# afb2001/path_planner

Hardware: AMD Instinct MI355X
Metric: Dubins edges costed/sec on 2048x2048 grid (higher is better)
Workload: dtype f64; 1 GPU; cfg3_2048_10pct_65536_obst16; grid=2048x2048 @0.1m, 10% blocked, samples_per_iter_per_gpu=65536, samples_per_iter_total=65536, dynamic_obstacles=16, obstacle_placement=uniform in the map (SURVEY 8d), seed 3, ribbons=5, heuristic=TspPointRobotNoSplitKRibbons K=2, edges_per_iter_per_gpu=236140

## Files before the change

### path_planner_amd/csrc/pp_k_common.h

```cpp
#pragma once
#include "../../include/ppgpu.h"
#include "pp_device.h"

struct __attribute__((aligned(128))) PPLaunchWords {
    unsigned need_big;
    unsigned live_count;
    unsigned hw_count;
    unsigned defer_count[PP_HL_MAX_N + 1];
    unsigned sweep_count;
    unsigned swept_total;
};
static_assert(sizeof(PPLaunchWords) == 128, "the launch counters share one 128-byte line");
static_assert(offsetof(PPLaunchWords, sweep_count) % 8 == 0 && offsetof(PPLaunchWords, swept_total) == offsetof(PPLaunchWords, sweep_count) + 4,
              "pp_k_mark_sweeps adds to sweep_count (low half) and swept_total (high half) with one 64-bit atomic");
__device__ __forceinline__ unsigned long long* pp_sweep_counters(PPLaunchWords* w) { return reinterpret_cast<unsigned long long*>(&w->sweep_count); }

struct PPParams {
    double max_speed, slow_speed, rho, rho_cov, horizon, tmin, inc_d, sst, ribw, cpf, tpf;
    double inv_inc_d;
    int heuristic, tsp_k;
    int fuse_h;
    int quiet_finish;
    int lane_split;
    int defer_h;
    double h_rho;
    PPGrid grid;
    const PPObst* obst; int n_obst; int obst_model;
    const ppgpu_vertex* verts; const double* ribbons; const double* tgrid; int ng; int nverts;
    const double* sx; const double* sy; const double* sh; long long n_samples;
    const unsigned long long* edges; long long n_edges;
    long long total_edges;
    const ppgpu_wrapper_edge* wedges;
    int v0, nv; long long s0, ns; unsigned cfg_mask; int per;
    ppgpu_edge_result* out; double* child; int stride;
    long long e_base, ws_base;
    struct PPEdgeSetup* setup;
    unsigned short* track_hits;
    unsigned long long* track_eq;
    unsigned* track_chunk_hits;
    double* track_pen;
    double* track_chunk_pen;
    struct PPTrackSummary* track_summary;
    unsigned char* track_skip;
    int2* track_far;
    unsigned long long* work;
    PPLaunchWords* words;
    int reset_words;
    unsigned* live_list;
    unsigned* defer_list;
    struct PPCoverState* cover_state;
    unsigned* hw_list;
    int ngp, nch;
    unsigned* share_head;
    unsigned* share_of;
    int approach_list;
    unsigned* sweep_list;
};

#define PP_SETUP_MALFORMED 1u
#define PP_SETUP_COLOCATED 2u
#define PP_SETUP_SHARED 4u
#define PP_SETUP_NO_SWEEP (PP_SETUP_MALFORMED | PP_SETUP_COLOCATED | PP_SETUP_SHARED)
#define PP_SHARE_KEYS 8
#define PP_SHARE_NONE 0xffffffffu
#define PP_FAR_DONE (-2)
#define PP_SHARE_UNSWEPT 0xfffffffeu
struct PPEdgeSetupBody {
    PPSegBase seg[3];
    double p0, p1, p2, hi1;
    double qx, qy, rho, rho_inv, length;
    double wStart, wEnd, speed;
    double approx;
    unsigned long long omask;
    int type;
    unsigned vi, cbits, sflags;
    double srcH;
};
struct __attribute__((aligned(128))) PPEdgeSetup : PPEdgeSetupBody {};
static_assert(sizeof(PPEdgeSetup) == 256 && sizeof(PPEdgeSetupBody) == 256, "PPEdgeSetup is sized for two 128-byte lines");
template <bool TAB = false>
__device__ __forceinline__ void pp_setup_seg_pose(const PPEdgeSetupBody* S, int i, double tprime, double p0, double p1, int word, double& ux, double& uy, double& uth) {
    const PPSegBase* g = &S->seg[i];
    pp_curve_seg<TAB>(pp_word_seg_type(word, i), (tprime - pp_seg_o1(i, p0)) - pp_seg_o2(i, p1), g->bx, g->by, g->bth, g->sb, g->cb, ux, uy, uth);
}
template <bool TAB = false>
__device__ __forceinline__ void pp_setup_seg_pose(const PPEdgeSetupBody* S, int i, double tprime, double& ux, double& uy, double& uth) {
    pp_setup_seg_pose<TAB>(S, i, tprime, S->p0, S->p1, S->type, ux, uy, uth);
}
#define PP_SETUP_GLOBAL_WORDS 32
#define PP_SETUP_WORDS 32
#define PP_SETUP_LDS_STRIDE 33
static_assert(sizeof(PPEdgeSetup) == 8 * PP_SETUP_GLOBAL_WORDS && sizeof(PPEdgeSetupBody) == 8 * PP_SETUP_WORDS, "the LDS staging of the skip planner copies whole records");

__global__ __launch_bounds__(256) void pp_k_grid_row_clear(const uint32_t* bits, int rows, int cols, int wpr, unsigned char* rowclear) {
    const long long i = (long long)blockIdx.x * 256 + threadIdx.x;
    if (i >= (long long)rows * cols) return;
    const int r = (int)(i / cols), c = (int)(i - (long long)r * cols);
    const uint32_t* row = bits + (size_t)r * wpr;
    int d = 0;
    for (; d < PP_CLEAR_CAP; d++) {
        const int a = c - d, b = c + d;
        if (a < 0 || b >= cols) break;
        if (((row[a >> 5] >> (a & 31)) | (row[b >> 5] >> (b & 31))) & 1u) break;
    }
    rowclear[i] = (unsigned char)d;
}
__global__ __launch_bounds__(256) void pp_k_grid_clear(const unsigned char* rowclear, int rows, int cols, unsigned char* clearance) {
    const long long i = (long long)blockIdx.x * 256 + threadIdx.x;
    if (i >= (long long)rows * cols) return;
    const int r = (int)(i / cols), c = (int)(i - (long long)r * cols);
    int best = rowclear[i];
    for (int dy = 1; dy < best; dy++) {
        const int up = r + dy, dn = r - dy;
        int m = dy;
        if (up < rows && dn >= 0) {
            const int ru = rowclear[(size_t)up * cols + c], rd = rowclear[(size_t)dn * cols + c];
            m = max(dy, min(ru, rd));
        }
        best = min(best, m);
    }
    clearance[i] = (unsigned char)best;
}

#define PP_TG_SEG 2048
__global__ __launch_bounds__(64) void pp_k_time_grid(const ppgpu_vertex* verts, int nverts, double sst, double inc_d, double max_speed,
                                                    int ng, double* tgrid) {
    __shared__ double seg[PP_TG_SEG];
    const int v = blockIdx.x;
    if (v >= nverts) return;
    const int lane = threadIdx.x;
    double timeIncrement = inc_d / max_speed;
    double t = verts[v].time;
    double timeSinceStart = t - sst;
    double timeNudge = fmod(timeSinceStart, timeIncrement);
    t += timeNudge;
    double* row = tgrid + (size_t)v * ng;
    int s = 0;
    for (int tries = 0; s < ng && tries < 8; tries++) {
        const double c = (t + timeIncrement) - t;
        int firstBad = ng;
        for (int k0 = s; k0 < ng; k0 += 64) {
            const int k = k0 + lane;
            const double val = t + (double)(k - s) * c;
            const double nxt = t + (double)(k + 1 - s) * c;
            if (k < ng) row[k] = val;
            const bool bad = (k < ng - 1) && !(val + timeIncrement == nxt);
            const unsigned long long m = __ballot(bad);
            if (m != 0ull) { firstBad = k0 + (int)__builtin_ctzll(m); break; }
        }
// ... 90 lines not shown
```

### path_planner_amd/csrc/pp_k_solve.h

```cpp
#pragma once
#ifndef PP_CR_SOLVE
#define PP_CR_SOLVE true
#endif
#ifndef PP_SOLVE_MIN_WAVES
#define PP_SOLVE_MIN_WAVES 1
#endif
__device__ __forceinline__ bool pp_edge_shareable(const PPParams& p, const PPCurve& cv, int type, unsigned sflags, unsigned cbits,
                                                  double wStart, double wEnd, double speed) {
    if (type < 0 || (sflags & (PP_SETUP_MALFORMED | PP_SETUP_COLOCATED)) || cbits >= 4u) return false;
    const double bound = p.horizon + 1e-12 + p.sst;
    if (wEnd < bound) return false;
    const double dist = (bound - wStart) * speed;
    if (!(dist <= cv.length)) return false;
    const double tprime = (cv.rho_inv != 0.0) ? dist * cv.rho_inv : dist / cv.rho;
    return tprime < cv.p0;
}
__device__ __forceinline__ unsigned pp_share_key(unsigned vi, unsigned cbits, int type) {
    return vi * PP_SHARE_KEYS + (cbits & 3u) * 2u + (pp_word_seg_type(type, 0) == 0 ? 0u : 1u);
}
__device__ __forceinline__ void pp_share_elect(const PPParams& p, bool member, unsigned key, unsigned pos) {
    bool pend = false;
    if (member) pend = pos < __hip_atomic_load(p.share_head + key, __ATOMIC_RELAXED, __HIP_MEMORY_SCOPE_AGENT);
    unsigned long long m;
    while ((m = __ballot(pend)) != 0ull) {
        const int leader = __ffsll((long long)m) - 1;
        const unsigned k0 = (unsigned)__builtin_amdgcn_readlane((int)key, leader);
        if (pp_lane() == leader) atomicMin(p.share_head + k0, pos);
        if (key == k0) pend = false;
    }
}

template <bool ALL_WORDS>
__device__ __forceinline__ void pp_solve_edges_body(const PPParams& p) {
    const long long e = (long long)blockIdx.x * 256 + threadIdx.x;
    pp_launch_reset(p, e);
    if (e >= p.n_edges) return;
    long long e2 = -1;
    if (!p.wedges && !p.edges) {
        const long long Q = p.total_edges / p.per;
        const int r = (int)((p.e_base + e) / Q);
        unsigned m = p.cfg_mask;
        for (int i = 0; i < p.per - 1 - r; i++) m &= m - 1;
        const unsigned c = (unsigned)(__ffs((int)m) - 1), c2 = c ^ PPGPU_EDGE_SLOW;
        if ((p.cfg_mask >> c2) & 1u) {
            const int r2 = (int)__popc(p.cfg_mask >> (c2 + 1));
            const long long ep = e + (long long)(r2 - r) * Q;
            if (ep >= 0 && ep < p.n_edges) {
                if (!(c & PPGPU_EDGE_SLOW)) return;
                e2 = ep;
            }
        }
    }
    unsigned vi, target, cbits;
    const long long eg = pp_edge_position(p, p.e_base + e);
    pp_edge_decode(p, eg, vi, target, cbits);
    PPCurve cv;
    bool valid = false;
    unsigned sflags = 0;
    double srcT = 0, wSpeed = 1, wStart = 0, wEnd = 0;
    double srcHeading = 0;
    PPDubins dub;
    dub.p0 = dub.p1 = dub.p2 = 0; dub.type = -1;
    if (vi >= (unsigned)p.nverts || (!p.wedges && (long long)target >= p.n_samples)) {
        sflags = PP_SETUP_MALFORMED;
        pp_curve_init<false>(cv, 0, 0, 0, 1.0, dub);
    } else {
        const ppgpu_vertex* V = p.verts + vi;
        const double srcX = V->x, srcY = V->y, srcH = V->heading;
        srcT = V->time;
        srcHeading = srcH;
        valid = true;
        double rho = (cbits & PPGPU_EDGE_COVERAGE) ? p.rho_cov : p.rho;
        if (p.wedges) {
            const ppgpu_wrapper_edge* W = p.wedges + eg;
            dub.p0 = W->param[0]; dub.p1 = W->param[1]; dub.p2 = W->param[2]; dub.type = W->type;
            if (dub.type < 0 || dub.type > 5) dub.type = -1;
            rho = W->rho; wSpeed = W->speed;
            pp_curve_init<PP_CR_SOLVE, PP_CR_SOLVE && !ALL_WORDS>(cv, W->qi[0], W->qi[1], W->qi[2], rho, dub);
            wStart = W->start_time; wEnd = W->end_time;
        } else {
            const double tgtX = p.sx[target], tgtY = p.sy[target], tgtH = p.sh[target];
            if ((srcX == tgtX) && (srcY == tgtY) && (srcH == tgtH)) sflags |= PP_SETUP_COLOCATED;
            if constexpr (ALL_WORDS || !PP_CR_SOLVE) {
                pp_dubins_shortest<PP_CR_SOLVE>(srcX, srcY, pp_yaw(srcH), tgtX, tgtY, pp_yaw(tgtH), rho, dub);
                pp_curve_init<PP_CR_SOLVE>(cv, srcX, srcY, pp_yaw(srcH), rho, dub);
            } else {
                pp_dubins_shortest_ranked(srcX, srcY, pp_yaw(srcH), tgtX, tgtY, pp_yaw(tgtH), rho, dub);
                pp_curve_init<PP_CR_SOLVE, true>(cv, srcX, srcY, pp_yaw(srcH), rho, dub);
            }
        }
        {
            const double bound = fabs(cv.qth) + cv.p0 + (cv.t1 == 1 ? 0.0 : cv.p1) + cv.p2;
            if (!(bound < 9.0e4)) dub.type = -1;
        }
    }
    bool member0 = false, member1 = false;
    unsigned key0 = 0u, key1 = 0u, pos0 = 0u, pos1 = 0u;
    for (int k = 0; k < (e2 >= 0 ? 2 : 1); k++) {
        PPEdgeSetup* __restrict__ O = p.setup + p.ws_base + (k ? e2 : e);
        struct { double approx, wStart, wEnd, speed; int type; unsigned vi, cbits, sflags; } S;
        S.vi = vi; S.cbits = k ? (cbits ^ PPGPU_EDGE_SLOW) : cbits; S.sflags = sflags; S.type = -1;
        S.approx = S.wStart = S.wEnd = 0; S.speed = 1;
        if (valid) {
            if (p.wedges) {
                S.speed = wSpeed;
                S.wStart = wStart; S.wEnd = wEnd;
                S.approx = (S.wEnd - srcT) * 1.0;
            } else {
                S.speed = (S.cbits & PPGPU_EDGE_SLOW) ? p.slow_speed : p.max_speed;
                S.approx = cv.length / S.speed * 1.0;
                S.wStart = srcT;
                S.wEnd = srcT + cv.length / S.speed;
            }
            S.type = dub.type;
        }
        if (p.share_head) {
            const long long egk = k ? pp_edge_position(p, p.e_base + e2) : eg;
            const bool member = pp_edge_shareable(p, cv, S.type, S.sflags, S.cbits, S.wStart, S.wEnd, S.speed);
            const bool unswept = S.type < 0 || (S.sflags & (PP_SETUP_MALFORMED | PP_SETUP_COLOCATED)) != 0u;
            const unsigned key = member ? pp_share_key(S.vi, S.cbits, S.type) : PP_SHARE_NONE;
            if (k) { member1 = member; key1 = key; pos1 = (unsigned)egk; } else { member0 = member; key0 = key; pos0 = (unsigned)egk; }
            p.share_of[egk] = unswept ? PP_SHARE_UNSWEPT : key;
        }
        pp_curve_segments(cv, O->seg);
        O->qx = cv.qx; O->qy = cv.qy; O->rho = cv.rho; O->rho_inv = cv.rho_inv; O->length = cv.length;
        O->p0 = cv.p0; O->p1 = cv.p1; O->p2 = cv.p2; O->hi1 = cv.p0 + cv.p1;
        O->approx = S.approx; O->wStart = S.wStart; O->wEnd = S.wEnd; O->speed = S.speed;
        O->type = S.type; O->vi = S.vi; O->cbits = S.cbits; O->sflags = S.sflags;
        O->srcH = srcHeading;
        unsigned long long omask = 0ull;
        if (p.n_obst > PP_WAVE) omask = ~0ull;
        else if (p.n_obst > 0 && S.type >= 0 && !(S.sflags & PP_SETUP_MALFORMED) && p.ng > 0) {
            const double t0 = p.tgrid[(size_t)vi * p.ng];
            const double endTime = fmin(p.horizon + 1e-12 + p.sst, S.wEnd);
            const double chunkTime = 64.0 * (p.inc_d / p.max_speed);
            const double duration = fmax(endTime - t0, 0.0) + chunkTime;
            const double travel = fmin(cv.length, fmax(endTime - S.wStart, 0.0) * S.speed) + 1e-3;
            for (int j = 0; j < p.n_obst; j++) {
                const PPObst& o = p.obst[j];
                const double dt = t0 - o.Time;
                const double X = o.X + o.Speed * dt * o.cosYaw, Y = o.Y + o.Speed * dt * o.sinYaw;
                const double R = o.reach + travel + fabs(o.Speed) * duration + 1e-3;
                const double dx = cv.qx - X, dy = cv.qy - Y;
                if (!(dx * dx + dy * dy > R * R)) omask |= 1ull << j;
            }
        }
        O->omask = omask;
    }
    if (p.share_head) {
        pp_share_elect(p, member0, key0, pos0);
        if (__ballot(e2 >= 0) != 0ull) pp_share_elect(p, member1, key1, pos1);
    }
}
#define PP_MARK_THREADS 1024
#define PP_MARK_THREADS_PLAIN 256
__global__ __launch_bounds__(PP_MARK_THREADS) void pp_k_mark_sweeps(PPParams p) {
    const long long e = (long long)blockIdx.x * blockDim.x + threadIdx.x;
    const bool valid = e < p.n_edges;
    const long long eg = valid ? pp_edge_position(p, p.e_base + e) : 0;
    const unsigned key = valid ? p.share_of[eg] : PP_SHARE_UNSWEPT;
    unsigned head = PP_SHARE_NONE;
    if (key != PP_SHARE_UNSWEPT && key != PP_SHARE_NONE) {
        head = p.share_head[key];
        if (head == (unsigned)eg) head = PP_SHARE_NONE;
    }
    const bool swept = key != PP_SHARE_UNSWEPT && head == PP_SHARE_NONE;
    unsigned at = 0u;
    if (p.sweep_list) {
        __shared__ unsigned s_cnt[PP_MARK_THREADS / 64];
        __shared__ unsigned s_base;
        const int lane = threadIdx.x & 63, wave = threadIdx.x >> 6;
        const unsigned long long m = __ballot(swept);
        if (lane == 0) s_cnt[wave] = (unsigned)__popcll(m);
        __syncthreads();
        if (threadIdx.x == 0) {
            unsigned tot = 0;
            for (int w = 0; w < (int)(blockDim.x >> 6); w++) tot += s_cnt[w];
            s_base = tot ? (unsigned)atomicAdd(pp_sweep_counters(p.words), ((unsigned long long)tot << 32) | tot) : 0u;
        }
        __syncthreads();
        at = s_base + (unsigned)__popcll(m & ((1ull << lane) - 1ull));
        for (int w = 0; w < wave; w++) at += s_cnt[w];
    }
    if (!valid) return;
    if (key != PP_SHARE_NONE) p.share_of[eg] = head;
    if (head != PP_SHARE_NONE) {
        PPEdgeSetup* S = p.setup + p.ws_base + e;
        S->sflags |= PP_SETUP_SHARED;
        double* r = reinterpret_cast<double*>(p.out + eg);
        const unsigned info = (unsigned)(S->type & 0xff);
        r[0] = __hiloint2double((int)info, 0);
        r[1] = 0.0; r[2] = 0.0; r[3] = S->approx;
        for (int i = 4; i < 13; i++) r[i] = 0.0;
        r[13] = S->p0; r[14] = S->p1; r[15] = S->p2;
    }
    if (!p.sweep_list) return;
    if (swept) p.sweep_list[at] = (unsigned)e;
    else {
        reinterpret_cast<int4*>(p.track_summary)[p.ws_base + e] = make_int4(0, 0, 0, 0);
        if (p.approach_list) {
            if (head != PP_SHARE_NONE) {
                p.track_far[p.ws_base + e] = make_int2(PP_FAR_DONE, 0);
            } else {
                p.track_far[p.ws_base + e] = make_int2(0, 0);
                const unsigned li = atomicAdd(&p.words->live_count, 1u);
                p.live_list[2 * (size_t)li] = (unsigned)e;
                p.live_list[2 * (size_t)li + 1] = (unsigned)eg;
            }
        }
    }
}
__global__ __launch_bounds__(256) void pp_k_share_fanout(PPParams p, int copy_child) {
    const long long eg = (long long)blockIdx.x * 16 + (threadIdx.x >> 4);
    const int sub = (int)(threadIdx.x & 15);
    if (eg >= p.n_edges) return;
    const unsigned h = p.share_of[eg];
    if (h == PP_SHARE_NONE) return;
    const unsigned long long* src = reinterpret_cast<const unsigned long long*>(p.out + h);
    unsigned long long* dst = reinterpret_cast<unsigned long long*>(p.out + eg);
    unsigned long long v = src[sub];
    if (sub == 0) v = (v & ~(0xffull << 32)) | (dst[0] & (0xffull << 32));
    if (sub != 3 && sub < 13) dst[sub] = v;
    if (copy_child) {
        const double* cs = p.child + (size_t)h * p.stride * 4;
        double* cd = p.child + (size_t)eg * p.stride * 4;
        for (int i = sub; i < p.stride * 4; i += 16) cd[i] = cs[i];
    }
}
__global__ __launch_bounds__(256, PP_SOLVE_MIN_WAVES) void pp_k_solve_edges(PPParams p) { pp_solve_edges_body<false>(p); }
__global__ __launch_bounds__(256, PP_SOLVE_MIN_WAVES) void pp_k_solve_edges_all_words(PPParams p) { pp_solve_edges_body<true>(p); }
```

### path_planner_amd/csrc/ppgpu.hip

```cpp
#include <hip/hip_runtime.h>

#include <algorithm>
#include <cfloat>
#include <cmath>
#include <cstdio>
#include <cstdlib>
#include <cstring>
#include <memory>
#include <mutex>
#include <string>
#include <vector>

#include "../../include/ppgpu.h"
#include "pp_kernels.h"
#include "pp_sampler.h"

static thread_local std::string g_err = "";
static int fail(int code, const std::string& msg) { g_err = msg; return code; }

#define HIP_TRY(call)                                                                              \
    do {                                                                                           \
        hipError_t _e = (call);                                                                    \
        if (_e != hipSuccess)                                                                      \
            return fail(PPGPU_EHIP, std::string(#call) + ": " + hipGetErrorString(_e));            \
// ... 79 lines not shown
enum { EV_BEGIN, EV_SOLVED, EV_POSED, EV_COVERED, EV_END, EV_APPROACHED, EV_COUNT };
struct ppgpu_ctx {
    int device = 0;
    hipStream_t own_stream = nullptr, stream = nullptr;
    hipStream_t side_stream = nullptr;
    hipEvent_t ev_fork = nullptr, ev_join = nullptr;
    bool have_cfg = false;
    ppgpu_config cfg{};
    DevBuf<uint32_t> grid;
    DevBuf<unsigned char> grid_clear, grid_rowclear;
    int rows = 0, cols = 0, wpr = 0;
    double res = 0;
    DevBuf<uint16_t> grid_dist;
    bool grid_dist_built = false;
    uint32_t keepout_limit2 = 0;
    DevBuf<uint32_t> grid_keepout;
    DevBuf<uint32_t> reach_labels;
    bool reach_labels_built = false;
    DevBuf<unsigned long long> reach_words;
    unsigned long long reach_free = 0, reach_components = 0, reach_cells = 0;
    bool reach_have_seed = false;
    double reach_seed_x = 0, reach_seed_y = 0;
    uint32_t reach_seed_label = PPGPU_REACH_NONE;
    bool reach_seed_fresh = false;
    DevBuf<uint32_t> reach_bits;
    DevBuf<uint16_t> reach_gap;
    bool reach_set_built = false;
    uint32_t reach_set_label = PPGPU_REACH_NONE;
    DevBuf<double> reach_ribbons;
    DevBuf<ppgpu_ribbon_reach_record> reach_records;
    TraceTimer t_reach_labels, t_reach_gap, t_reach_ribbons;
    DevBuf<PPObst> obst;
    int n_obst = 0;
    int obst_model = PPGPU_OBST_NONE;
    DevBuf<ppgpu_vertex> verts;
    DevBuf<double> ribbons, tgrid;
    int nverts = 0, nribbons = 0, ng = 0;
    DevBuf<double> sx, sy, sh;
    long long n_samples = 0;
    long long n_extra = 0;
    PPSamplerState sampler{};
    DevBuf<double> samp_ribbons;
    DevBuf<unsigned long long> samp_pos;
    int samp_group = -1;
    unsigned long long* pinned_counts = nullptr;
    std::vector<double> samp_ribbons_host;
    DevBuf<unsigned char> s_bytes;
    DevBuf<unsigned long long> s_u64;
    DevBuf<unsigned> s_u32a, s_u32b;
    DevBuf<double> s_cand;
    DevBuf<unsigned long long> tmp_edges, partial;
    DevBuf<ppgpu_wrapper_edge> tmp_wedges;
    DevBuf<ppgpu_edge_result> tmp_results;
    DevBuf<double> tmp_child, tmp_lengths, tmp_len_out, int_child;
    DevBuf<unsigned char> tmp_trace;
    DevBuf<ppgpu_cover_summary> tmp_summaries;
    DevBuf<double> tmp_cover_child;
    DevBuf<int> tmp_counts;
    TraceTimer t_steps, t_cover, t_contacts, t_clearance;
    TraceTimer t_tsp;
    TraceTimer t_dist;
    TraceTimer t_keepout;
    bool quiet_finish = true;
    bool solve_all_words = false;
    bool lane_split = true;
    bool lane_finish = true;
    bool plan_spans = true;
    bool lane_heuristic = true;
    long long prepass_min_edges = PP_PREPASS_MIN_EDGES;
    bool share_sweeps = true;
    bool use_sweep_list = true;
    bool approach_list = true;
    size_t slice_bytes = PP_SLICE_BYTES;
    DevBuf<PPEdgeSetup> setup;
    DevBuf<unsigned short> track_hits;
    DevBuf<unsigned long long> track_eq;
    DevBuf<unsigned> track_chunk_hits;
    DevBuf<PPTrackSummary> track_summary;
    DevBuf<int2> track_far;
    DevBuf<unsigned char> track_skip;
    DevBuf<PPLaunchWords> words;
    DevBuf<unsigned> defer_list, live_list, hw_list;
    DevBuf<unsigned> share_head, share_of;
    bool last_launch_shared = false;
    DevBuf<unsigned> sweep_list;
    long long last_launch_slices = 0, last_slice_edges = 0;
    bool last_launch_listed = false;
    DevBuf<PPCoverState> cover_state;
    DevBuf<unsigned long long> work;
    int n_cu = 0;
    int resident[2] = {0, 0};
    DevBuf<double> track_pen, track_chunk_pen;
    bool timing = false;
    hipEvent_t ev_ring[PP_TIMING_RING][EV_COUNT] = {};
    double ms_ring[PP_TIMING_RING][4] = {};
    int ev_slot = 0;
    long long last_launch_edges = 0;
    bool last_launch_packed = false;
    long long live_earlier_slices = 0;
    long long ev_launches = 0;
    int max_vertex_ribbons = 0;
    DevBuf<int> tmp_idx;
    ExpandWork expand;
    unsigned long long order_fallbacks = 0;
    DevBuf<unsigned char> dstage_in, dstage_out;
    void* stage_in = nullptr; size_t stage_in_cap = 0;
    void* stage_out = nullptr; size_t stage_out_cap = 0;
    DevBuf<unsigned long long> gather;
    void* comm = nullptr;
    unsigned long long hsa_gpu = 0, hsa_cpu = 0, hsa_signal = 0;
    bool copy_pending = false;
    int tsp_table_min = 0, tsp_table_max = 0;
    int tsp_dubins_min = 0, tsp_dubins_max = 0;
    int tsp_table_cap = 0;
    DevBuf<unsigned char> tsp_slots;
    DevBuf<unsigned> tsp_list;
    DevBuf<double> tsp_T;
    DevBuf<unsigned long long> tsp_words;

    __attribute__((visibility("hidden"))) ~ppgpu_ctx() {
        for (void* pinned : {(void*)pinned_counts, stage_in, stage_out}) if (pinned) (void)hipHostFree(pinned);
        for (auto& set : ev_ring) for (hipEvent_t e : set) if (e) (void)hipEventDestroy(e);
        for (hipEvent_t e : {t_steps.ev[0], t_steps.ev[1], t_cover.ev[0], t_cover.ev[1], t_contacts.ev[0], t_contacts.ev[1], t_clearance.ev[0], t_clearance.ev[1], t_tsp.ev[0], t_tsp.ev[1], t_dist.ev[0], t_dist.ev[1], t_keepout.ev[0], t_keepout.ev[1],
                             t_reach_labels.ev[0], t_reach_labels.ev[1], t_reach_gap.ev[0], t_reach_gap.ev[1], t_reach_ribbons.ev[0], t_reach_ribbons.ev[1], ev_fork, ev_join}) if (e) (void)hipEventDestroy(e);
        for (hipStream_t s : {side_stream, own_stream}) if (s) (void)hipStreamDestroy(s);
    }
};

static int require_cfg(ppgpu_ctx* c) {
    if (!c) return fail(PPGPU_EINVAL, "null context");
    if (!c->have_cfg) return fail(PPGPU_ESTATE, "ppgpu_set_config must be called first");
    return PPGPU_OK;
}

static int require_vertices(ppgpu_ctx* c) {
    int rc = require_cfg(c);
    if (rc) return rc;
    if (c->nverts <= 0) return fail(PPGPU_ESTATE, "ppgpu_set_vertices must be called (after ppgpu_set_config)");
    return PPGPU_OK;
}

static int require_world(ppgpu_ctx* c) {
    int rc = require_vertices(c);
    if (rc) return rc;
    if (c->n_samples + c->n_extra <= 0) return fail(PPGPU_ESTATE, "no targets: call ppgpu_sampler_add, ppgpu_set_samples or ppgpu_set_extra_targets");
    return PPGPU_OK;
}

static int check_open_vertices(const ppgpu_ctx* c, const char* who, int n, const ppgpu_vertex* hv, int n_ribbons, int* max_ribbons) {
    *max_ribbons = 0;
    for (int i = 0; i < n; i++) {
        if (hv[i].ribbon_count < 0 || hv[i].ribbon_offset < 0 || hv[i].ribbon_offset + hv[i].ribbon_count > n_ribbons)
            return fail(PPGPU_EINVAL, std::string(who) + ": ribbon range outside the pool");
        if (hv[i].ribbon_count > PP_WAVE) return fail(PPGPU_ECAPACITY, std::string(who) + ": more than 64 ribbons on one vertex");
        if (hv[i].time < c->cfg.start_state_time) return fail(PPGPU_EINVAL, std::string(who) + ": vertex time before start_state_time");
        if (hv[i].ribbon_count > *max_ribbons) *max_ribbons = hv[i].ribbon_count;
    }
    return PPGPU_OK;
}

static int check_wrapper_edges(const ppgpu_ctx* c, const char* who, int64_t n, const ppgpu_wrapper_edge* w) {
    for (int64_t i = 0; i < n; i++) {
        if (!(w[i].rho > 0) || !(w[i].speed > 0)) return fail(PPGPU_EINVAL, std::string(who) + ": rho and speed must be positive");
        if (w[i].vertex < 0 || w[i].vertex >= c->nverts) return fail(PPGPU_EINVAL, std::string(who) + ": vertex out of range");
    }
    return PPGPU_OK;
// ... 1061 lines not shown
    HIP_TRY(hipMemcpyAsync(&fb, c->expand.fallbacks.p, sizeof(unsigned), hipMemcpyDeviceToHost, c->stream));
    HIP_TRY(hipStreamSynchronize(c->stream));
    c->order_fallbacks += fb;
    if (h_fallbacks) *h_fallbacks = fb;
    return PPGPU_OK;
}

uint64_t ppgpu_order_fallbacks(ppgpu_ctx* c) { return c ? c->order_fallbacks : 0; }

int64_t ppgpu_dense_edge_count(int32_t nv, int64_t ns, uint32_t cfg_mask) {
    return (int64_t)nv * ns * (int64_t)__builtin_popcount(cfg_mask & 0xFu);
}

static unsigned resident_grid(ppgpu_ctx* c, bool gaussian, long long n_edges) {
    int& resident = c->resident[gaussian ? 1 : 0];
    if (resident == 0) {
        const void* kernel = gaussian ? (const void*)pp_k_cover_sweep_gaussian : (const void*)pp_k_cover_sweep;
        int per_cu = 0;
        if (hipOccupancyMaxActiveBlocksPerMultiprocessor(&per_cu, kernel, PP_WPB * 64, 0) != hipSuccess || per_cu <= 0) per_cu = 2;
        resident = per_cu * (c->n_cu > 0 ? c->n_cu : 256);
    }
    const long long need = (n_edges + PP_WPB - 1) / PP_WPB;
    return (unsigned)(need < resident ? need : resident);
}

static PPParams list_params(ppgpu_ctx* c, long long n, const unsigned long long* d_edges, const ppgpu_wrapper_edge* d_wedges,
                            ppgpu_edge_result* d_out, double* d_child, int stride) {
    PPParams p;
    fill_params(c, p);
    p.edges = d_edges; p.wedges = d_wedges;
    p.v0 = 0; p.nv = 0; p.s0 = 0; p.ns = 1; p.cfg_mask = 0; p.per = 1;
    p.n_edges = n;
    p.out = d_out; p.child = d_child; p.stride = stride;
    return p;
}

struct CostLaunch {
    PPParams p;
    bool gaussian;
    bool prepasses;
    bool skip_chunks;
    bool packed;
    bool lane_finish;
    bool fuse_h;
    bool defer_h;
    bool quiet_finish, lane_split;
    bool forked;
    bool share;
    bool share_child;
    bool sweep_list;
    int nch, ngp;
    long long slice;
};

static void cost_modes(const ppgpu_ctx* c, CostLaunch& m) {
    const PPParams& p = m.p;
    const long long total = p.n_edges;
    m.gaussian = p.n_obst > 0 && p.obst_model == PPGPU_OBST_GAUSSIAN;
    m.nch = (p.ng + PP_WAVE - 1) / PP_WAVE;
    if (m.nch < 1) m.nch = 1;
    m.ngp = m.nch * PP_WAVE;
    const size_t per_edge = sizeof(PPEdgeSetup) + (size_t)m.ngp * sizeof(unsigned short) +
                            (size_t)m.nch * (sizeof(unsigned long long) + sizeof(unsigned)) + sizeof(PPTrackSummary) +
                            (m.gaussian ? (size_t)(m.ngp + m.nch) * sizeof(double) : 0);
    m.slice = (long long)(c->slice_bytes / per_edge);
    if (m.slice < PP_WPB) m.slice = PP_WPB;
    if (m.slice > total) m.slice = total;
    m.prepasses = total >= c->prepass_min_edges;
    m.skip_chunks = m.prepasses && !p.wedges && (c->rows == 0 || c->grid_clear.p) && p.ng >= PP_WAVE;
    const bool dubinsH = p.heuristic == PPGPU_H_TSP_DUBINS_ALL || p.heuristic == PPGPU_H_TSP_DUBINS_K;
    m.fuse_h = PP_FUSE_HEUR && !dubinsH && !m.gaussian;
    m.defer_h = m.fuse_h && m.prepasses && c->lane_heuristic && total < (1ll << 32) &&
                (p.heuristic == PPGPU_H_TSP_POINT_ALL || p.heuristic == PPGPU_H_TSP_POINT_K);
    m.quiet_finish = m.prepasses && c->quiet_finish;
    m.lane_split = m.prepasses && c->lane_split && !m.gaussian;
    m.packed = m.prepasses && total < (1ll << 32);
#if defined(PP_DBG_COUNTS)
    const bool laneFinishBuilt = false;
#else
    const bool laneFinishBuilt = true;
#endif
    m.lane_finish = laneFinishBuilt && m.packed && c->lane_finish && !m.gaussian;
    m.forked = m.lane_finish && m.fuse_h && p.heuristic != PPGPU_H_MAX_DISTANCE;
    m.share = m.prepasses && m.packed && !p.wedges && c->share_sweeps && (long long)p.nverts * PP_SHARE_KEYS < (1ll << 32);
    m.share_child = m.share && p.child != nullptr;
    m.sweep_list = m.share && c->use_sweep_list;
}

static int cost_workspace(ppgpu_ctx* c, CostLaunch& m) {
    PPParams& p = m.p;
    const size_t total = (size_t)p.n_edges, ws = (size_t)m.slice;
    hipStream_t st = c->stream;
    int rc;
    if (!p.child) {
        int stride = c->max_vertex_ribbons + 8;
        if (stride > PP_WAVE) stride = PP_WAVE;
        if ((rc = c->int_child.reserve(total * stride * 4, false, st))) return rc;
        p.child = c->int_child.p;
        p.stride = stride;
    }
    p.nch = m.nch; p.ngp = m.ngp;
    if ((rc = c->setup.reserve(ws, false, st)) || (rc = c->track_hits.reserve(ws * p.ngp, false, st)) ||
        (rc = c->track_eq.reserve(ws * p.nch, false, st)) || (rc = c->track_chunk_hits.reserve(ws * p.nch, false, st)) ||
        (rc = c->track_summary.reserve(ws, false, st)) || (rc = c->track_far.reserve(ws, false, st)) ||
        (rc = c->track_skip.reserve(ws * p.nch, false, st)))
        return rc;
    if (m.gaussian && ((rc = c->track_pen.reserve(ws * p.ngp, false, st)) || (rc = c->track_chunk_pen.reserve(ws * p.nch, false, st))))
        return rc;
    if ((rc = c->words.reserve(1, false, st)) || (rc = c->work.reserve(PP_WORK_WORDS, false, st))) return rc;
    p.setup = c->setup.p; p.track_hits = c->track_hits.p; p.track_eq = c->track_eq.p;
    p.track_chunk_hits = c->track_chunk_hits.p; p.track_summary = c->track_summary.p;
    p.track_far = m.prepasses ? c->track_far.p : nullptr;
    p.track_skip = m.skip_chunks ? c->track_skip.p : nullptr;
    p.track_pen = c->track_pen.p; p.track_chunk_pen = c->track_chunk_pen.p;
    p.words = c->words.p; p.reset_words = 1;
    p.work = c->work.p;
    p.fuse_h = m.fuse_h; p.defer_h = m.defer_h; p.quiet_finish = m.quiet_finish; p.lane_split = m.lane_split;
    if (m.packed) {
        if ((rc = c->live_list.reserve(ws * 2, false, st))) return rc;
        p.live_list = c->live_list.p;
    }
    if (m.lane_finish) {
        if ((rc = c->cover_state.reserve(ws, false, st)) || (rc = c->hw_list.reserve(total, false, st))) return rc;
        p.cover_state = c->cover_state.p; p.hw_list = c->hw_list.p;
    }
    if (m.defer_h) {
        if ((rc = c->defer_list.reserve(total * PP_HL_MAX_N, false, st))) return rc;
        p.defer_list = c->defer_list.p;
    }
    if (m.share) {
        if ((rc = c->share_head.reserve((size_t)p.nverts * PP_SHARE_KEYS, false, st)) || (rc = c->share_of.reserve(total, false, st))) return rc;
        p.share_head = c->share_head.p; p.share_of = c->share_of.p;
    }
    if (m.sweep_list) {
        if ((rc = c->sweep_list.reserve(ws + PP_WPB, false, st))) return rc;
        p.sweep_list = c->sweep_list.p;
        p.approach_list = c->approach_list ? 1 : 0;
    }
    return PPGPU_OK;
}

static int bank_slice_timing(ppgpu_ctx* c, bool packed) {
    hipEvent_t* ev = c->ev_ring[c->ev_slot];
    HIP_TRY(hipEventSynchronize(ev[EV_COVERED]));
    float ms[4] = {0, 0, 0, 0};
    int rc = slice_durations(ev, ms);
    if (rc) return rc;
    for (int i = 0; i < 4; i++) c->ms_ring[c->ev_slot][i] += ms[i];
    if (packed) { unsigned live = 0; HIP_TRY(hipMemcpy(&live, &c->words.p->live_count, sizeof(unsigned), hipMemcpyDeviceToHost)); c->live_earlier_slices += live; }
    return PPGPU_OK;
}

static int cost_slice(ppgpu_ctx* c, const CostLaunch& m) {
    const PPParams& p = m.p;
    hipStream_t st = c->stream;
    hipEvent_t* ev = c->ev_ring[c->ev_slot];
    if (c->timing) HIP_TRY(hipEventRecord(ev[EV_BEGIN], st));
    hipLaunchKernelGGL(c->solve_all_words ? pp_k_solve_edges_all_words : pp_k_solve_edges, dim3((unsigned)((p.n_edges + 255) / 256)), dim3(256), 0, st, p);
    if (m.share) {
        const unsigned mark_threads = m.sweep_list ? PP_MARK_THREADS : PP_MARK_THREADS_PLAIN;
        hipLaunchKernelGGL(pp_k_mark_sweeps, dim3((unsigned)((p.n_edges + mark_threads - 1) / mark_threads)), dim3(mark_threads), 0, st, p);
    }
    if (c->timing) HIP_TRY(hipEventRecord(ev[EV_SOLVED], st));
    if (m.skip_chunks) {
        int epw = 256 / p.nch;
        if (epw < 1) epw = 1;
        if (epw > PP_PLAN_EDGES_MAX) epw = PP_PLAN_EDGES_MAX;
        const unsigned blocks = (unsigned)((p.n_edges + epw - 1) / epw);
        const bool many = p.n_obst > PP_WAVE;
        void (*planner)(PPParams, int);
        if (m.sweep_list) planner = m.gaussian ? (many ? pp_k_plan_skips_gaussian_many : (c->plan_spans ? pp_k_plan_skips_gaussian : pp_k_plan_skips_gaussian_chunkwise))
                                               : (many ? pp_k_plan_skips_many : (c->plan_spans ? pp_k_plan_skips : pp_k_plan_skips_chunkwise));
        else planner = m.gaussian ? (many ? pp_k_plan_skips_gaussian_many_direct : (c->plan_spans ? pp_k_plan_skips_gaussian_direct : pp_k_plan_skips_gaussian_chunkwise_direct))
                                  : (many ? pp_k_plan_skips_many_direct : (c->plan_spans ? pp_k_plan_skips_direct : pp_k_plan_skips_chunkwise_direct));
        hipLaunchKernelGGL(planner, dim3(blocks, (unsigned)((epw * p.nch + 255) / 256)), dim3(256), 0, st, p, epw);
    }
    void (*pose)(PPParams) = m.sweep_list ? (m.gaussian ? pp_k_pose_sweep_gaussian : pp_k_pose_sweep) : (m.gaussian ? pp_k_pose_sweep_gaussian_direct : pp_k_pose_sweep_direct);
    hipLaunchKernelGGL(pose, dim3((unsigned)((p.n_edges + PP_WPB - 1) / PP_WPB)), dim3(PP_WPB * 64), 0, st, p);
    if (c->timing) HIP_TRY(hipEventRecord(ev[EV_POSED], st));
    if (m.prepasses) hipLaunchKernelGGL(p.approach_list ? pp_k_approach_events : pp_k_approach_events_direct, dim3((unsigned)((p.n_edges + PP_APPROACH_THREADS - 1) / PP_APPROACH_THREADS)), dim3(PP_APPROACH_THREADS), 0, st, p);
    if (c->timing) HIP_TRY(hipEventRecord(ev[EV_APPROACHED], st));
    hipLaunchKernelGGL(m.gaussian ? pp_k_cover_sweep_gaussian : pp_k_cover_sweep, dim3(resident_grid(c, m.gaussian, p.n_edges)), dim3(PP_WPB * 64), 0, st, p);
    if (m.lane_finish)
        hipLaunchKernelGGL(pp_k_cover_finish, dim3((unsigned)((p.n_edges + PP_FINISH_THREADS - 1) / PP_FINISH_THREADS)), dim3(PP_FINISH_THREADS), 0, st, p);
    if (c->timing) HIP_TRY(hipEventRecord(ev[EV_COVERED], st));
    return PPGPU_OK;
}

static int tsp_table_pass(ppgpu_ctx* c, const PPParams& p) {
    const bool point = p.heuristic == PPGPU_H_TSP_POINT_ALL || p.heuristic == PPGPU_H_TSP_POINT_K;
    const bool dubins = p.heuristic == PPGPU_H_TSP_DUBINS_ALL || p.heuristic == PPGPU_H_TSP_DUBINS_K;
    if (!point && !dubins) return PPGPU_OK;
    const int range_min = dubins ? c->tsp_dubins_min : c->tsp_table_min, range_max = dubins ? c->tsp_dubins_max : c->tsp_table_max;
    if (range_max <= 0 || !p.child || p.stride <= 0 || p.n_edges <= 0) return PPGPU_OK;
    hipStream_t st = c->stream;
    PPTspTableArgs q;
    q.out = p.out; q.child = p.child; q.stride = p.stride; q.n_edges = p.n_edges;
    q.heuristic = p.heuristic; q.tsp_k = p.tsp_k; q.ribw = p.ribw; q.max_speed = p.max_speed; q.tpf = p.tpf; q.h_rho = p.h_rho;
    q.min_ribbons = range_min; q.max_ribbons = range_max;
    q.list = c->tsp_list.p; q.list_cap = (unsigned)c->tsp_list.cap; q.count = (unsigned*)(c->tsp_words.p + 2); q.stats = c->tsp_words.p;
    q.slots = c->tsp_slots.p; q.bytes = c->tsp_slots.cap;
    q.T = dubins ? c->tsp_T.p : nullptr;
    if (dubins && q.list_cap > PP_TT_TCAP) q.list_cap = PP_TT_TCAP;
    if (c->timing) HIP_TRY(hipEventRecord(c->t_tsp.ev[0], st));
    HIP_TRY(hipMemsetAsync(c->tsp_words.p + 2, 0, sizeof(unsigned long long), st));
    hipLaunchKernelGGL(pp_k_tsp_table_list, dim3((unsigned)((p.n_edges + 255) / 256)), dim3(256), 0, st, q);
    const long long grid = p.n_edges < PP_TT_GRID ? p.n_edges : PP_TT_GRID;
    if (dubins) hipLaunchKernelGGL(pp_k_tsp_table_dubins_T, dim3((unsigned)grid), dim3(256), 0, st, q);
    hipLaunchKernelGGL(dubins ? pp_k_tsp_table_dubins : pp_k_tsp_table, dim3((unsigned)grid), dim3(PP_TT_THREADS), 0, st, q);
    if (c->timing) { HIP_TRY(hipEventRecord(c->t_tsp.ev[1], st)); c->t_tsp.ms_earlier = 0; c->t_tsp.timed = true; }
    return PPGPU_OK;
}

static int cost_heuristic_tail(ppgpu_ctx* c, const CostLaunch& m) {
    const PPParams& p = m.p;
    const long long total = p.n_edges;
    hipStream_t st = c->stream;
    const dim3 per_wave((unsigned)((total + PP_H_WPB - 1) / PP_H_WPB));
    if (p.heuristic == PPGPU_H_TSP_DUBINS_ALL || p.heuristic == PPGPU_H_TSP_DUBINS_K)
        hipLaunchKernelGGL(pp_k_heuristic_dubins, per_wave, dim3(PP_H_WPB * 64), 0, st, p);
    else if (!m.fuse_h)
        hipLaunchKernelGGL(pp_k_heuristic, per_wave, dim3(PP_H_WPB * 64), 0, st, p);
    if (m.forked) {
        HIP_TRY(hipEventRecord(c->ev_fork, st));
        HIP_TRY(hipStreamWaitEvent(c->side_stream, c->ev_fork, 0));
        hipLaunchKernelGGL(pp_k_heuristic_listed, per_wave, dim3(PP_H_WPB * 64), 0, c->side_stream, p);
        HIP_TRY(hipEventRecord(c->ev_join, c->side_stream));
    }
    if (m.defer_h) {
        hipLaunchKernelGGL(pp_k_deferred_list, dim3((unsigned)((total + 256 * PP_DL_PER - 1) / (256 * PP_DL_PER))), dim3(256), 0, st, p);
        hipLaunchKernelGGL(pp_k_heuristic_lanes, dim3((unsigned)((total * PP_HL_SPLIT + PP_HL_THREADS - 1) / PP_HL_THREADS) + PP_HL_MAX_N), dim3(PP_HL_THREADS), 0, st, p);
    }
    if (p.heuristic == PPGPU_H_TSP_POINT_K)
        hipLaunchKernelGGL(pp_k_heuristic_big, dim3((unsigned)(total < PP_BIG_GRID ? total : PP_BIG_GRID)), dim3(PP_BIG_WPB * 64), 0, st, p);
    if (m.forked) HIP_TRY(hipStreamWaitEvent(st, c->ev_join, 0));
    int rc = tsp_table_pass(c, p);
    if (rc) return rc;
    if (m.share) hipLaunchKernelGGL(pp_k_share_fanout, dim3((unsigned)((total + 15) / 16)), dim3(256), 0, st, p, m.share_child ? 1 : 0);
    return PPGPU_OK;
}

static int launch_cost(ppgpu_ctx* c, const PPParams& asked, CostLaunch* done = nullptr) {
    CostLaunch local;
    CostLaunch& m = done ? *done : local;
    m.p = asked;
    PPParams& p = m.p;
    const long long total = p.n_edges;
    if (total <= 0) return PPGPU_OK;
    p.total_edges = total;
    if ((total + PP_WPB - 1) / PP_WPB > 0x3fffffffll) return fail(PPGPU_ECAPACITY, "cost_edges: too many edges for one launch");
    cost_modes(c, m);
    int rc = cost_workspace(c, m);
    if (rc) return rc;
    if (c->timing) c->ev_slot = (int)(c->ev_launches % PP_TIMING_RING);
    for (double& ms : c->ms_ring[c->ev_slot]) ms = 0;
    c->live_earlier_slices = 0;
    c->last_launch_shared = false; c->last_launch_listed = false;
    if (m.share) HIP_TRY(hipMemsetAsync(p.share_head, 0xff, (size_t)p.nverts * PP_SHARE_KEYS * sizeof(unsigned), c->stream));
    c->last_launch_slices = 0;
    for (long long e0 = 0; e0 < total; e0 += m.slice) {
        p.e_base = e0; p.ws_base = 0; p.n_edges = (total - e0 < m.slice) ? (total - e0) : m.slice;
        c->last_launch_slices++; c->last_slice_edges = p.n_edges;
        if (c->timing && e0 > 0 && (rc = bank_slice_timing(c, m.packed))) return rc;
        if ((rc = cost_slice(c, m))) return rc;
    }
    p.e_base = 0;
    p.n_edges = total;
    if ((rc = cost_heuristic_tail(c, m))) return rc;
    c->last_launch_edges = total; c->last_launch_packed = m.packed; c->last_launch_shared = m.share; c->last_launch_listed = m.sweep_list;
    if (c->timing) { HIP_TRY(hipEventRecord(c->ev_ring[c->ev_slot][EV_END], c->stream)); c->ev_launches++; }
    HIP_TRY(hipGetLastError());
    return PPGPU_OK;
}

int ppgpu_cost_edges_dense(ppgpu_ctx* c, int32_t v0, int32_t nv, int64_t s0, int64_t ns, uint32_t cfg_mask,
                           ppgpu_edge_result* d_results, double* d_child, int32_t stride) {
    int rc = require_world(c);
    if (rc) return rc;
    HIP_TRY(hipSetDevice(c->device));
    cfg_mask &= 0xFu;
    if (v0 < 0 || nv <= 0 || v0 + nv > c->nverts) return fail(PPGPU_EINVAL, "cost_edges_dense: vertex range");
    if (s0 < 0 || ns <= 0 || s0 + ns > c->n_samples) return fail(PPGPU_EINVAL, "cost_edges_dense: sample range");
    if (!cfg_mask || !d_results) return fail(PPGPU_EINVAL, "cost_edges_dense: empty configuration mask or null results");
    if (d_child && stride <= 0) return fail(PPGPU_EINVAL, "cost_edges_dense: ribbon_stride must be positive");
    PPParams p;
    fill_params(c, p);
    p.edges = nullptr; p.wedges = nullptr;
    p.v0 = v0; p.nv = nv; p.s0 = s0; p.ns = ns; p.cfg_mask = cfg_mask; p.per = __builtin_popcount(cfg_mask);
    p.n_edges = (long long)nv * ns * p.per;
    p.out = d_results; p.child = d_child; p.stride = stride;
    return launch_cost(c, p);
}

int ppgpu_cost_edges_list(ppgpu_ctx* c, int64_t n, const uint64_t* d_edges, ppgpu_edge_result* d_results, double* d_child,
                          int32_t stride) {
    int rc = require_world(c);
    if (rc) return rc;
    HIP_TRY(hipSetDevice(c->device));
    if (n < 0 || (n > 0 && (!d_edges || !d_results))) return fail(PPGPU_EINVAL, "cost_edges_list: bad arguments");
    if (d_child && stride <= 0) return fail(PPGPU_EINVAL, "cost_edges_list: ribbon_stride must be positive");
    return launch_cost(c, list_params(c, n, (const unsigned long long*)d_edges, nullptr, d_results, d_child, stride));
}

enum TraceKind { TRACE_STEPS, TRACE_COVER, TRACE_CONTACTS, TRACE_CLEARANCE };
struct TraceRequest {
    TraceKind kind;
    int32_t stride;
    int32_t* counts;
    void* records;
    size_t rec_bytes;
    ppgpu_cover_summary* summaries;
    double* child;
    int32_t ribbon_stride;
    uint32_t limit2;
};
static TraceRequest steps_request(int32_t stride, int32_t* counts, ppgpu_step_record* steps) {
    return TraceRequest{TRACE_STEPS, stride, counts, steps, sizeof(ppgpu_step_record), nullptr, nullptr, 0, 0};
}
static TraceRequest cover_request(int32_t stride, int32_t* counts, ppgpu_cover_record* cover, ppgpu_cover_summary* summaries, double* child, int32_t ribbon_stride) {
    return TraceRequest{TRACE_COVER, stride, counts, cover, sizeof(ppgpu_cover_record), summaries, child, ribbon_stride, 0};
}
static TraceRequest contacts_request(int32_t* counts, ppgpu_contact_record* contacts) {
    return TraceRequest{TRACE_CONTACTS, 0, counts, contacts, sizeof(ppgpu_contact_record), nullptr, nullptr, 0, 0};
}
static TraceRequest clearance_request(int32_t* counts, ppgpu_clearance_record* clearance, uint32_t limit2) {
    return TraceRequest{TRACE_CLEARANCE, 1, counts, clearance, sizeof(ppgpu_clearance_record), nullptr, nullptr, 0, limit2};
}
static int clearance_limit2(const ppgpu_ctx* c, const char* who, double margin, uint32_t* limit2) {
    *limit2 = 0;
    if (c->rows == 0 || !(margin > 0)) return PPGPU_OK;
    if (ppgpu_keepout_limit2(c->res, margin, limit2)) return fail(PPGPU_EINVAL, std::string(who) + ": margin above 255 cells");
    return PPGPU_OK;
}

static int trace_request_args(const ppgpu_ctx* c, const char* who, bool device, int64_t n, const void* edges, const void* results, const TraceRequest& r) {
    static const char* const records_name[] = {"d_steps", "d_cover", "d_contacts", "d_clearance"};
    const bool cover = r.kind == TRACE_COVER, contacts = r.kind == TRACE_CONTACTS;
    if (n < 0 || (n > 0 && (!edges || !r.counts || ((!contacts || c->n_obst > 0) && !r.records)))) return fail(PPGPU_EINVAL, std::string(who) + ": bad arguments");
    if (!contacts && (r.stride <= 0 || r.stride > 65535)) return fail(PPGPU_EINVAL, std::string(who) + ": step_stride must be in 1 .. 65535");
    if (device) {
        if (n > 0 && (!results || (cover && !r.summaries))) return fail(PPGPU_EINVAL, std::string(who) + (cover ? ": null results or summaries" : ": null results"));
    } else if (cover && n > 0 && !r.summaries) {
        return fail(PPGPU_EINVAL, std::string(who) + ": null summaries");
    }
    if (cover && r.child && r.ribbon_stride <= 0) return fail(PPGPU_EINVAL, std::string(who) + ": ribbon_stride must be positive");
    if (device && ((unsigned long long)r.records & 15ull) != 0ull)
        return fail(PPGPU_EINVAL, std::string(who) + ": " + records_name[r.kind] + " must be 16-byte aligned");
    return PPGPU_OK;
}

static void trace_kernel(ppgpu_ctx* c, const CostLaunch& L, const PPParams& q, const TraceRequest& r, void* dst, long long rec_base) {
    const dim3 grid((unsigned)((q.n_edges + PP_TRACE_WPB - 1) / PP_TRACE_WPB)), block(PP_TRACE_WPB * 64);
    switch (r.kind) {
    case TRACE_STEPS:
// ... 778 lines not shown
```

Measured before the change: 189.5 million edges/s.

## Stage share-head election in LDS and pad table entries to avoid atomic contention

The sweep-sharing election now does its atomicMin first in a 64-slot per-block LDS table, then flushes one global atomic per slot after a barrier. Global share_head entries are padded to 32 words each so different keys sit in different cache lines. The table is reset in the fanout kernel rather than by a host memset each launch. The aim is fewer contended global atomics and no per-launch memset. The cost is a 32x larger table, extra block barriers, and a tighter size limit that can disable sharing on big graphs.

New measurement: 196.7 million edges/s (median of 6 runs). 3.8% higher.

```diff
diff --git a/path_planner_amd/csrc/pp_k_common.h b/path_planner_amd/csrc/pp_k_common.h
--- a/path_planner_amd/csrc/pp_k_common.h
+++ b/path_planner_amd/csrc/pp_k_common.h
@@ -65,6 +65,8 @@
 #define PP_SHARE_NONE 0xffffffffu
 #define PP_FAR_DONE (-2)
 #define PP_SHARE_UNSWEPT 0xfffffffeu
+#define PP_SHARE_STRIDE 32u
+__device__ __forceinline__ unsigned* pp_share_entry(const PPParams& p, unsigned key) { return p.share_head + (size_t)key * PP_SHARE_STRIDE; }
 struct PPEdgeSetupBody {
     PPSegBase seg[3];
     double p0, p1, p2, hi1;
diff --git a/path_planner_amd/csrc/pp_k_solve.h b/path_planner_amd/csrc/pp_k_solve.h
--- a/path_planner_amd/csrc/pp_k_solve.h
+++ b/path_planner_amd/csrc/pp_k_solve.h
@@ -18,22 +18,34 @@
 __device__ __forceinline__ unsigned pp_share_key(unsigned vi, unsigned cbits, int type) {
     return vi * PP_SHARE_KEYS + (cbits & 3u) * 2u + (pp_word_seg_type(type, 0) == 0 ? 0u : 1u);
 }
-__device__ __forceinline__ void pp_share_elect(const PPParams& p, bool member, unsigned key, unsigned pos) {
+#define PP_ELECT_SLOTS 64
+struct PPElectLds { unsigned key[PP_ELECT_SLOTS], pos[PP_ELECT_SLOTS]; };
+__device__ __forceinline__ void pp_share_elect_wave(const PPParams& p, PPElectLds& lds, bool member, unsigned key, unsigned pos) {
     bool pend = false;
-    if (member) pend = pos < __hip_atomic_load(p.share_head + key, __ATOMIC_RELAXED, __HIP_MEMORY_SCOPE_AGENT);
+    if (member) pend = pos < __hip_atomic_load(pp_share_entry(p, key), __ATOMIC_RELAXED, __HIP_MEMORY_SCOPE_AGENT);
     unsigned long long m;
     while ((m = __ballot(pend)) != 0ull) {
         const int leader = __ffsll((long long)m) - 1;
         const unsigned k0 = (unsigned)__builtin_amdgcn_readlane((int)key, leader);
-        if (pp_lane() == leader) atomicMin(p.share_head + k0, pos);
+        if (pp_lane() == leader) {
+            const unsigned slot = k0 & (PP_ELECT_SLOTS - 1u);
+            const unsigned was = atomicCAS(&lds.key[slot], PP_SHARE_NONE, k0);
+            if (was == PP_SHARE_NONE || was == k0) atomicMin(&lds.pos[slot], pos);
+            else atomicMin(pp_share_entry(p, k0), pos);
+        }
         if (key == k0) pend = false;
     }
 }
+__device__ __forceinline__ void pp_share_elect_flush(const PPParams& p, const PPElectLds& lds) {
+    if (threadIdx.x >= PP_ELECT_SLOTS) return;
+    const unsigned k = lds.key[threadIdx.x], pos = lds.pos[threadIdx.x];
+    if (k == PP_SHARE_NONE) return;
+    if (pos < __hip_atomic_load(pp_share_entry(p, k), __ATOMIC_RELAXED, __HIP_MEMORY_SCOPE_AGENT)) atomicMin(pp_share_entry(p, k), pos);
+}
+struct PPElectAsk { bool member0, member1, two; unsigned key0, key1, pos0, pos1; };
 
 template <bool ALL_WORDS>
-__device__ __forceinline__ void pp_solve_edges_body(const PPParams& p) {
-    const long long e = (long long)blockIdx.x * 256 + threadIdx.x;
-    pp_launch_reset(p, e);
+__device__ __forceinline__ void pp_solve_edge_records(const PPParams& p, long long e, PPElectAsk& ask) {
     if (e >= p.n_edges) return;
     long long e2 = -1;
     if (!p.wedges && !p.edges) {
@@ -147,9 +159,28 @@
         }
         O->omask = omask;
     }
+    ask.member0 = member0; ask.key0 = key0; ask.pos0 = pos0;
+    ask.member1 = member1; ask.key1 = key1; ask.pos1 = pos1;
+    ask.two = e2 >= 0;
+}
+template <bool ALL_WORDS>
+__device__ __forceinline__ void pp_solve_edges_body(const PPParams& p) {
+    __shared__ PPElectLds lds;
+    const long long e = (long long)blockIdx.x * 256 + threadIdx.x;
+    pp_launch_reset(p, e);
     if (p.share_head) {
-        pp_share_elect(p, member0, key0, pos0);
-        if (__ballot(e2 >= 0) != 0ull) pp_share_elect(p, member1, key1, pos1);
+        if (threadIdx.x < PP_ELECT_SLOTS) { lds.key[threadIdx.x] = PP_SHARE_NONE; lds.pos[threadIdx.x] = PP_SHARE_NONE; }
+        __syncthreads();
+    }
+    PPElectAsk ask;
+    ask.member0 = ask.member1 = ask.two = false;
+    ask.key0 = ask.key1 = PP_SHARE_NONE; ask.pos0 = ask.pos1 = 0u;
+    pp_solve_edge_records<ALL_WORDS>(p, e, ask);
+    if (p.share_head) {
+        pp_share_elect_wave(p, lds, ask.member0, ask.key0, ask.pos0);
+        if (__ballot(ask.two) != 0ull) pp_share_elect_wave(p, lds, ask.member1, ask.key1, ask.pos1);
+        __syncthreads();
+        pp_share_elect_flush(p, lds);
     }
 }
 #define PP_MARK_THREADS 1024
@@ -161,7 +192,7 @@
     const unsigned key = valid ? p.share_of[eg] : PP_SHARE_UNSWEPT;
     unsigned head = PP_SHARE_NONE;
     if (key != PP_SHARE_UNSWEPT && key != PP_SHARE_NONE) {
-        head = p.share_head[key];
+        head = *pp_share_entry(p, key);
         if (head == (unsigned)eg) head = PP_SHARE_NONE;
     }
     const bool swept = key != PP_SHARE_UNSWEPT && head == PP_SHARE_NONE;
@@ -211,6 +242,9 @@
     }
 }
 __global__ __launch_bounds__(256) void pp_k_share_fanout(PPParams p, int copy_child) {
+    const unsigned long long n_keys = (unsigned long long)p.nverts * PP_SHARE_KEYS;
+    for (unsigned long long k = (unsigned long long)blockIdx.x * 256u + threadIdx.x; k < n_keys; k += (unsigned long long)gridDim.x * 256u)
+        *pp_share_entry(p, (unsigned)k) = PP_SHARE_NONE;
     const long long eg = (long long)blockIdx.x * 16 + (threadIdx.x >> 4);
     const int sub = (int)(threadIdx.x & 15);
     if (eg >= p.n_edges) return;
diff --git a/path_planner_amd/csrc/ppgpu.hip b/path_planner_amd/csrc/ppgpu.hip
--- a/path_planner_amd/csrc/ppgpu.hip
+++ b/path_planner_amd/csrc/ppgpu.hip
@@ -185,6 +185,7 @@
     DevBuf<PPLaunchWords> words;
     DevBuf<unsigned> defer_list, live_list, hw_list;
     DevBuf<unsigned> share_head, share_of;
+    bool share_head_stale = true;
     bool last_launch_shared = false;
     DevBuf<unsigned> sweep_list;
     long long last_launch_slices = 0, last_slice_edges = 0;
@@ -1412,7 +1413,7 @@
 #endif
     m.lane_finish = laneFinishBuilt && m.packed && c->lane_finish && !m.gaussian;
     m.forked = m.lane_finish && m.fuse_h && p.heuristic != PPGPU_H_MAX_DISTANCE;
-    m.share = m.prepasses && m.packed && !p.wedges && c->share_sweeps && (long long)p.nverts * PP_SHARE_KEYS < (1ll << 32);
+    m.share = m.prepasses && m.packed && !p.wedges && c->share_sweeps && (long long)p.nverts * PP_SHARE_KEYS * PP_SHARE_STRIDE <= (1ll << 26);
     m.share_child = m.share && p.child != nullptr;
     m.sweep_list = m.share && c->use_sweep_list;
 }
@@ -1459,7 +1460,9 @@
         p.defer_list = c->defer_list.p;
     }
     if (m.share) {
-        if ((rc = c->share_head.reserve((size_t)p.nverts * PP_SHARE_KEYS, false, st)) || (rc = c->share_of.reserve(total, false, st))) return rc;
+        const unsigned* const table_was = c->share_head.p;
+        if ((rc = c->share_head.reserve((size_t)p.nverts * PP_SHARE_KEYS * PP_SHARE_STRIDE, false, st)) || (rc = c->share_of.reserve(total, false, st))) return rc;
+        if (c->share_head.p != table_was) c->share_head_stale = true;
         p.share_head = c->share_head.p; p.share_of = c->share_of.p;
     }
     if (m.sweep_list) {
@@ -1586,7 +1589,10 @@
     for (double& ms : c->ms_ring[c->ev_slot]) ms = 0;
     c->live_earlier_slices = 0;
     c->last_launch_shared = false; c->last_launch_listed = false;
-    if (m.share) HIP_TRY(hipMemsetAsync(p.share_head, 0xff, (size_t)p.nverts * PP_SHARE_KEYS * sizeof(unsigned), c->stream));
+    if (m.share) {
+        if (c->share_head_stale) HIP_TRY(hipMemsetAsync(c->share_head.p, 0xff, c->share_head.cap * sizeof(unsigned), c->stream));
+        c->share_head_stale = true;
+    }
     c->last_launch_slices = 0;
     for (long long e0 = 0; e0 < total; e0 += m.slice) {
         p.e_base = e0; p.ws_base = 0; p.n_edges = (total - e0 < m.slice) ? (total - e0) : m.slice;
@@ -1600,6 +1606,7 @@
     c->last_launch_edges = total; c->last_launch_packed = m.packed; c->last_launch_shared = m.share; c->last_launch_listed = m.sweep_list;
     if (c->timing) { HIP_TRY(hipEventRecord(c->ev_ring[c->ev_slot][EV_END], c->stream)); c->ev_launches++; }
     HIP_TRY(hipGetLastError());
+    if (m.share) c->share_head_stale = false;
     return PPGPU_OK;
 }
 
```
